# HumanCompatibleAI/overcooked_ai

Measured on NVIDIA H100. Metric: env-steps/sec (joint transitions), higher is better.
Workload: dtype int32

## Files before the change

overcooked_ai_b200/csrc/ovc_rollout.cuh:

```cuda
#pragma once

namespace ovc {

struct Derived {
    uint16_t face[1024];
    uint8_t move[2048];
    int32_t cook5[32];
    int32_t deliver5[32];
    uint8_t potcode5[32][2];
    uint8_t dcode5[32];
    uint8_t pad[32];
};
static_assert(sizeof(Derived) == 4480, "Derived table size");
constexpr int DERIVED_ZERO_CHUNKS = (1024 * 2 + 2048) / 16;
#define OVC_DOFF(field) ((uint32_t)offsetof(Derived, field))
#define OVC_LOFF(field) ((uint32_t)offsetof(ovc_layout_t, field))

constexpr unsigned POT_FROZEN = 1u << 31;
constexpr int ROLLOUT_MAX_STEPS = 1 << 22;

__device__ __forceinline__ unsigned lds_tile(uint32_t a) {
    unsigned v;
    asm volatile("ld.shared.u32 %0, [%1];" : "=r"(v) : "r"(a) : "memory");
    return v;
}
__device__ __forceinline__ void sts_tile(uint32_t a, unsigned v) { asm volatile("st.shared.u32 [%0], %1;" ::"r"(a), "r"(v) : "memory"); }
__device__ __forceinline__ int4 lds_tile4(uint32_t a) {
    int4 v;
    asm volatile("ld.shared.v4.u32 {%0, %1, %2, %3}, [%4];" : "=r"(v.x), "=r"(v.y), "=r"(v.z), "=r"(v.w) : "r"(a) : "memory");
    return v;
}
__device__ __forceinline__ void sts_tile4(uint32_t a, int4 v) {
    asm volatile("st.shared.v4.u32 [%0], {%1, %2, %3, %4};" ::"r"(a), "r"(v.x), "r"(v.y), "r"(v.z), "r"(v.w) : "memory");
}
__device__ __forceinline__ unsigned lds_tbl32(uint32_t a) {
    unsigned v;
    asm volatile("ld.shared.u32 %0, [%1];" : "=r"(v) : "r"(a));
    return v;
}
__device__ __forceinline__ unsigned lds_tbl16(uint32_t a) {
    unsigned short v;
    asm volatile("ld.shared.u16 %0, [%1];" : "=h"(v) : "r"(a));
    return v;
}
__device__ __forceinline__ unsigned lds_tbl8(uint32_t a) {
    unsigned v;
    asm volatile("ld.shared.u8 %0, [%1];" : "=r"(v) : "r"(a));
    return v;
}

__device__ __forceinline__ int recipe_row5(unsigned k5) {
    const int n = k5 & 3;
    const int nt = __popc((k5 >> 2) & ((1u << n) - 1u));
    return ((n - nt) << 2) | nt;
}

__device__ __forceinline__ unsigned code_mask_of(int c) {
    if (c == 0) return 0u;
    if (c <= 6) {
        const int b = (0x0A0005 >> (((c - 1) >> 1) * 8)) & 0xFF;
        return (1u << b) | ((unsigned)((c - 1) & 1) << (b + 1));
    }
    if (c == 7) return 1u << OVC_EV_SOUP_PICKUP;
    if (c <= 13) {
        const int b = (0x0C0207 >> (((c - 8) >> 1) * 8)) & 0xFF;
        return (1u << b) | ((unsigned)((c - 8) & 1) << (b + 1));
    }
    if (c == 14) return 1u << OVC_EV_SOUP_DROP;
    if (c <= 22) {
        const int tom = (c - 15) >> 2, cls = (c - 15) & 3;
        const unsigned base = 1u << (tom ? OVC_EV_POTTING_TOMATO : OVC_EV_POTTING_ONION);
        const unsigned opt = 1u << (OVC_EV_OPTIMAL_ONION_POTTING + tom), via = 1u << (OVC_EV_VIABLE_ONION_POTTING + tom);
        const unsigned cat = 1u << (OVC_EV_CATASTROPHIC_ONION_POTTING + tom), usl = 1u << (OVC_EV_USELESS_ONION_POTTING + tom);
        return base | (cls == 0 ? (opt | via) : cls == 1 ? via : cls == 2 ? cat : (opt | usl));
    }
    const unsigned row = (unsigned)((0xC98654321ull >> ((c - 23) * 4)) & 15u);
    return (1u << OVC_EV_SOUP_DELIVERY) | (row << OVC_EV_RECIPE_SHIFT);
}

template <int S, int SWZ>
struct TileRec {
    uint32_t rec;
    uint32_t xm;
    __device__ __forceinline__ TileRec(uint32_t tile, int tid) {
        rec = tile + (uint32_t)tid * S * 4;
        if (SWZ == 0) xm = 0;
        else if (S <= 32) xm = ((((uint32_t)tid * S * 4) >> 7) & ((1u << SWZ) - 1u)) << 4;
        else xm = (uint32_t)tid * (S / 32);
    }
    __device__ __forceinline__ uint32_t phys(uint32_t off) const {
        if (SWZ == 0) return off;
        if (S <= 32) return off ^ xm;
        return off ^ (((xm + (off >> 7)) & 7u) << 4);
    }
    __device__ __forceinline__ int4 ld4(int c) const { return lds_tile4(rec + phys((uint32_t)c * 16)); }
    __device__ __forceinline__ void st4(int c, int4 v) const { sts_tile4(rec + phys((uint32_t)c * 16), v); }
    __device__ __forceinline__ uint32_t addr(int w) const { return rec + phys((uint32_t)w * 4); }
    __device__ __forceinline__ unsigned ldw(int w) const { return lds_tile(addr(w)); }
    __device__ __forceinline__ void stw(int w, unsigned v) const { sts_tile(addr(w), v); }
};

__device__ __forceinline__ unsigned pot_to_chip(unsigned w, uint32_t D, unsigned clk) {
    const unsigned tp1 = (w >> 8) & 0x3FFFu;
    if ((w & 7u) != OVC_O_SOUP || tp1 == 0) return w & 0x3FFFFFu;
    const unsigned cook = lds_tbl32(D + OVC_DOFF(cook5) + 4u * ((w >> 3) & 31u));
    if (tp1 - 1u > cook) return (w & 0x3FFFFFu) | POT_FROZEN;
    return (w & 0xFFu) | ((clk + (cook - (tp1 - 1u)) + 1u) << 8);
}
__device__ __forceinline__ unsigned pot_to_ext(unsigned w, uint32_t D, unsigned clk) {
    if (w & POT_FROZEN) return w & 0x3FFFFFu;
    const unsigned g = w >> 8;
    if (g == 0) return w;
    const unsigned cook = lds_tbl32(D + OVC_DOFF(cook5) + 4u * ((w >> 3) & 31u));
    const unsigned left = g - 1u > clk ? g - 1u - clk : 0u;
    return (w & 0xFFu) | ((cook - left + 1u) << 8);
}

struct RollOut {
    int sparse, sh0, sh1;
    unsigned c0, c1;
};

constexpr unsigned PS_FULL = 1u, PS_DISH = 1u << 4;
template <class R>
__device__ __forceinline__ unsigned pot_summary(const R &r, int n_pots) {
    unsigned ps = 0;
#pragma unroll 1
    for (int k = 0; k < n_pots; k++) {
        const unsigned w = r.ldw(4 + k);
        const bool soup = (w & 7u) == OVC_O_SOUP;
        const bool idle = (w >> 8) == 0;
        const unsigned n = (w >> 3) & 3u;
        if (soup && (!idle || n == 3u)) ps += PS_FULL;
        if (soup && (!idle || n == 1u || n == 2u)) ps += PS_DISH;
    }
    return ps;
}

template <class R>
__device__ __forceinline__ unsigned interact_v2(const R &r, uint32_t L, uint32_t D, unsigned &me, const unsigned other_t,
                                                unsigned &misc, const unsigned ps, unsigned &psn, const int n_pots,
                                                const bool old_dyn, const unsigned s, int &sparse, int &shaped) {
    const unsigned cell = lds_tbl16(D + OVC_DOFF(face) + 2u * (me & 0x3FFu));
    const unsigned terr = cell & 7u;
    unsigned held = me >> 10;
    const unsigned ht = held & 7u;
    unsigned code = 0;
    if (terr - 1u < 4u) {
        const bool ctr = terr == OVC_T_COUNTER;
        const uint32_t wa = r.addr(4 + (int)(cell >> 8));
        unsigned cw = terr - 1u;
        if (ctr) cw = lds_tile(wa);
        const bool pick = held == 0 && cw != 0;
        const bool drop = ctr && held != 0 && cw == 0;
        if (pick || drop) {
            const unsigned ot = (held | cw) & 7u;
            const unsigned n_full = ps & 15u;
            bool u;
            if (ot == OVC_O_DISH)
                u = pick ? ((misc & 0xFF00u) == 0 && (other_t == OVC_O_DISH ? 1u : 0u) < (ps >> 4)) : (n_full == 0 && other_t != OVC_O_ONION);
            else
                u = ot <= OVC_O_TOMATO && pick != (n_full == (unsigned)n_pots && other_t != OVC_O_DISH);
            code = 2u * ot + (pick ? 0xFFFFFFFFu : 6u) + (unsigned)u;
            if (ctr) {
                sts_tile(wa, held);
                if (ot == OVC_O_DISH) misc += pick ? 0xFFFFFF00u : 0x100u;
            } else {
                if (ot == OVC_O_TOMATO) code = 0;
                if (ot == OVC_O_DISH && u) shaped += (int)lds_tbl32(L + OVC_LOFF(rew_dish_pickup));
            }
            held = pick ? cw : 0u;
        }
    } else if (terr == OVC_T_POT) {
        const uint32_t wa = r.addr(4 + (int)(cell >> 8));
        const unsigned w = lds_tile(wa);
        const unsigned k5 = (w >> 3) & 31u;
        const unsigned n = k5 & 3u;
        if (ht == 0) {
            if (!old_dyn && (w & ~0xF8u) == OVC_O_SOUP && n != 0) {
                sts_tile(wa, w | ((s + lds_tbl32(D + OVC_DOFF(cook5) + 4u * k5) + 1u) << 8));
                psn += n == 3u ? PS_DISH : PS_FULL;
            }
        } else if (ht == OVC_O_DISH) {
            const unsigned g = w >> 8;
            if ((int)w < 0 || g - 1u <= s) {
                code = 7;
                held = pot_to_ext(w, D, s);
                sts_tile(wa, 0u);
                shaped += (int)lds_tbl32(L + OVC_LOFF(rew_soup_pickup));
                psn -= PS_FULL + PS_DISH;
            }
        } else if (ht <= OVC_O_TOMATO) {
            if ((w >> 8) == 0 && n < 3u) {
                const unsigned tom = ht == OVC_O_TOMATO;
                code = lds_tbl8(D + OVC_DOFF(potcode5) + 2u * k5 + tom);
                sts_tile(wa, ((w ? w : (unsigned)OVC_O_SOUP) + 8u) | (tom << (5 + n)));
                shaped += (int)lds_tbl32(L + OVC_LOFF(rew_placement_in_pot));
                held = 0;
                psn += n == 0 ? PS_DISH : n == 2u ? PS_FULL - PS_DISH : 0u;
            }
        }
    } else if (terr == OVC_T_SERVE && ht == OVC_O_SOUP) {
        const unsigned k5 = (held >> 3) & 31u;
        sparse += (int)lds_tbl32(D + OVC_DOFF(deliver5) + 4u * k5);
        code = lds_tbl8(D + OVC_DOFF(dcode5) + k5);
        held = 0;
    }
    me = (me & 0x3FFu) | (held << 10);
    return code;
}

constexpr int FMT_WIDE = 0, FMT_HOST = 1, FMT_STREAM = 2;

template <int FMT>
struct RollIO {
    static constexpr bool WIDE = FMT == FMT_WIDE;
    const StepArgs &a;
    unsigned oi, ai;
    const unsigned n;
    unsigned live_mask, cnt, cap, lane_lt, mi, n_groups;
    unsigned short *vals;
    bool leader;
    __device__ __forceinline__ RollIO(const StepArgs &args, long long env, unsigned live) : a(args), n((unsigned)args.n_envs) {
        oi = ai = (unsigned)env;
        live_mask = live, cnt = 0, cap = 0, lane_lt = 0, mi = 0, n_groups = 0, vals = nullptr, leader = false;
        if (FMT == FMT_STREAM) {
            n_groups = (unsigned)((a.n_envs + 31) >> 5);
            mi = (unsigned)(env >> 5);
            cap = ((unsigned)a.flags >> OVC_F_STREAM_CAP_SHIFT) & 0xFFFFu;
            const unsigned lane = (unsigned)env & 31u;
            lane_lt = (1u << lane) - 1u, leader = lane == 0;
            vals = reinterpret_cast<unsigned short *>(a.sparse) + (size_t)mi * cap;
        }
    }
    __device__ __forceinline__ int2 load_action() const {
        if (!WIDE && (a.flags & OVC_F_ACT_PACKED)) {
            const unsigned u = reinterpret_cast<const unsigned char *>(a.actions)[ai];
            return make_int2((int)(u & 15u), (int)(u >> 4));
        }
        if (!WIDE && (a.flags & OVC_F_ACT_U8)) {
            const uchar2 u = reinterpret_cast<const uchar2 *>(a.actions)[ai];
            return make_int2(u.x, u.y);
        }
        return reinterpret_cast<const int2 *>(a.actions)[ai];
    }
    __device__ __forceinline__ void next_action() { ai += n; }
    __device__ __forceinline__ void write(const RollOut &o, int done_v, bool stepped, uint32_t mask) {
        const unsigned i = oi;
        oi += n;
        if (FMT == FMT_STREAM) {
            const unsigned w = o.c0 | (o.c1 << 5) | ((unsigned)done_v << 10) | (stepped ? 1u << 11 : 0u) |
                               (o.sh0 != 0 ? 1u << 12 : 0u) | (o.sh1 != 0 ? 1u << 13 : 0u);
            const unsigned m = __ballot_sync(live_mask, w != 0);
            if (leader) reinterpret_cast<unsigned *>(a.events)[mi] = m;
            mi += n_groups;
            if (w != 0) {
                const unsigned pos = cnt + __popc(m & lane_lt);
                if (pos < cap) vals[pos] = (unsigned short)w;
            }
            cnt += __popc(m);
            if (a.done) reinterpret_cast<unsigned short *>(a.done)[i] = (unsigned short)w;
            return;
        }
        if (!WIDE && (a.flags & (OVC_F_OUT_CODES | OVC_F_OUT_PACKED))) {
            unsigned w = o.c0 | (o.c1 << 5) | ((unsigned)done_v << 10) | (stepped ? 1u << 11 : 0u);
            if (a.flags & OVC_F_OUT_CODES) {
                w |= (o.sh0 != 0 ? 1u << 12 : 0u) | (o.sh1 != 0 ? 1u << 13 : 0u);
            } else {
                reinterpret_cast<short *>(a.sparse)[i] = (short)o.sparse;
                reinterpret_cast<char2 *>(a.shaped)[i] = make_char2((signed char)o.sh0, (signed char)o.sh1);
            }
            reinterpret_cast<unsigned short *>(a.events)[i] = (unsigned short)w;
            return;
        }
        const unsigned e0 = stepped ? (unsigned)OVC_EVF_STEPPED_DONE : lds_tbl32(mask + 4u * o.c0);
        const unsigned e1 = stepped ? (unsigned)OVC_EVF_STEPPED_DONE : lds_tbl32(mask + 4u * o.c1);
        if (!WIDE && (a.flags & OVC_F_OUT_NARROW)) {
            reinterpret_cast<short *>(a.sparse)[i] = (short)o.sparse;
            reinterpret_cast<unsigned char *>(a.done)[i] = (unsigned char)done_v;
            reinterpret_cast<char2 *>(a.shaped)[i] = make_char2((signed char)o.sh0, (signed char)o.sh1);
        } else {
            a.sparse[i] = o.sparse;
            a.done[i] = done_v;
            reinterpret_cast<int2 *>(a.shaped)[i] = make_int2(o.sh0, o.sh1);
        }
        reinterpret_cast<int2 *>(a.events)[i] = make_int2((int)e0, (int)e1);
    }
};

template <int S, int TILE>
struct RollCfg {
    static constexpr int ROW_WORDS = S == 16 ? 16 : 32;
    static constexpr int ROWS_PER_ENV = S / ROW_WORDS;
    static constexpr int BOX_ROWS = TILE * ROWS_PER_ENV;
    static constexpr int SWZ = S == 16 ? 2 : 3;
    static constexpr int TILE_BYTES = TILE * S * 4;
    static_assert(BOX_ROWS <= 256, "TMA box rows");
    static_assert(TILE_BYTES % 1024 == 0, "tile must keep the swizzle alignment of what follows");
    static size_t smem_bytes(int n_layouts) { return (size_t)TILE_BYTES + (size_t)n_layouts * (sizeof(ovc_layout_t) + sizeof(Derived)) + 128 + 16; }
};

template <int S, int TILE, bool RS, int FMT>
__global__ void __launch_bounds__(TILE)
rollout_kernel(const __grid_constant__ CUtensorMap tmap, const StepArgs a) {
    using C = RollCfg<S, TILE>;
    constexpr bool WIDE = FMT == FMT_WIDE;
    const int tid = threadIdx.x;
    const long long env0 = (long long)blockIdx.x * TILE;
    const long long env = env0 + tid;
    const bool live = env < a.n_envs;
    const int T = a.n_steps;
    const int n_tbl = a.n_layouts;

    extern __shared__ __align__(1024) char smem[];
    char *tile = smem;
    ovc_layout_t *tbl = reinterpret_cast<ovc_layout_t *>(smem + C::TILE_BYTES);
    Derived *der = reinterpret_cast<Derived *>(smem + C::TILE_BYTES + (size_t)n_tbl * sizeof(ovc_layout_t));
    unsigned *mask = reinterpret_cast<unsigned *>(reinterpret_cast<char *>(der) + (size_t)n_tbl * sizeof(Derived));
    uint64_t *bar = reinterpret_cast<uint64_t *>(mask + 32);
    const uint32_t tbl_bytes = (uint32_t)n_tbl * (uint32_t)sizeof(ovc_layout_t);

    if (tid == 0) {
        mbar_init(bar, 1);
        mbar_expect_tx(bar, (uint32_t)C::TILE_BYTES + tbl_bytes);
        prefetch_tmap(&tmap);
        bulk_load_1d(tbl, a.layouts, tbl_bytes, bar);
    }
    for (int l = 0; l < n_tbl; l++)
        for (int i = tid; i < DERIVED_ZERO_CHUNKS; i += TILE) reinterpret_cast<int4 *>(der + l)[i] = make_int4(0, 0, 0, 0);
    if (tid < 32) mask[tid] = code_mask_of(tid);
    asm volatile("griddepcontrol.wait;" ::: "memory");
    if (tid == 0) tma_load_2d(tile, &tmap, 0, (int)(env0 * C::ROWS_PER_ENV), bar);
    int2 act = make_int2(OVC_A_STAY, OVC_A_STAY);
    if (live) act = load_action<WIDE>(a, env);
    __syncthreads();
    mbar_wait(bar, 0);
    asm volatile("griddepcontrol.launch_dependents;" ::: "memory");

    for (int l = 0; l < n_tbl; l++) {
        const ovc_layout_t *L = tbl + l;
        Derived *D = der + l;
        if (tid < 32) {
            const unsigned k5 = tid;
            const int n = k5 & 3, row = recipe_row5(k5);
            D->cook5[k5] = L->cook_time[row];
            D->deliver5[k5] = L->deliver_value[row];
            D->dcode5[k5] = (uint8_t)(23u + (unsigned)((0x0008007605432100ull >> (row * 4)) & 15u));
            const int old_val = L->best_value[n ? row : 0];
#pragma unroll
            for (int tom = 0; tom < 2; tom++) {
                int cls = 0;
                if (n < 3) {
                    const int new_val = L->best_value[recipe_row5((k5 + 1u) | ((unsigned)tom << (2 + n)))];
                    cls = new_val > 0 ? (old_val == new_val ? 0 : 1) : (old_val > 0 ? 2 : 3);
                }
                D->potcode5[k5][tom] = (uint8_t)(15 + 4 * tom + cls);
            }
        }
        const int n_free = L->n_free;
        for (int i = tid; i < n_free * 12; i += TILE) {
            const int f = i / 12, d = i - f * 12;
            const int pos = L->free_pos[f];
            if (d < 4) {
                D->face[(d << 8) | pos] = L->cell[(pos + dir_delta(d)) & 0xFF];
            } else {
                const int act_i = d - 4;
                int np = pos;
                if (act_i < 4) {
                    const int tp = (pos + dir_delta(act_i)) & 0xFF;
                    if ((L->cell[tp] & 7) == OVC_T_FLOOR) np = tp;
                }
                D->move[(act_i << 8) | pos] = (uint8_t)np;
            }
        }
    }
    __syncthreads();

    const unsigned live_mask = __ballot_sync(0xFFFFFFFFu, live);
    if (live) {
        const TileRec<S, C::SWZ> r(smem_u32(tile), tid);
        const uint32_t tbl_s = smem_u32(tbl), der_s = smem_u32(der), mask_s = smem_u32(mask);
        int t;
        unsigned toff;
        unsigned p0, p1, misc, ps, psn;
        uint32_t L, D;
        int n_pots;
        bool old_dyn;
        auto load_regs = [&](unsigned clk) {
            const int4 h = r.ld4(0);
            t = h.x, p0 = (unsigned)h.y, p1 = (unsigned)h.z, misc = (unsigned)h.w;
            toff = clk - (unsigned)t;
            unsigned lid = misc & 0xFFu;
            if (lid >= (unsigned)n_tbl) lid = 0;
            L = tbl_s + lid * (uint32_t)sizeof(ovc_layout_t), D = der_s + lid * (uint32_t)sizeof(Derived);
            n_pots = (int)lds_tbl32(L + OVC_LOFF(n_pots));
            old_dyn = (lds_tbl32(L + OVC_LOFF(flags)) & OVC_LAYOUT_OLD_DYNAMICS) != 0;
#pragma unroll 1
            for (int k = 0; k < n_pots; k++) r.stw(4 + k, pot_to_chip(r.ldw(4 + k), D, clk));
            ps = psn = pot_summary(r, n_pots);
        };
        load_regs(0u);

        RollIO<FMT> io(a, env, live_mask);

        auto interact = [&](bool second, RollOut &o) {
            unsigned pa = second ? p1 : p0;
            const unsigned pb = second ? p0 : p1;
            int sh = 0;
            const unsigned c = interact_v2(r, L, D, pa, (pb >> 10) & 7u, misc, ps, psn, n_pots, old_dyn, (unsigned)t + toff, o.sparse, sh);
            if (second) p1 = pa, o.sh1 = sh, o.c1 = c;
            else p0 = pa, o.sh0 = sh, o.c0 = c;
        };
        auto finish = [&](int a0, int a1, const RollOut &o, bool stepped) {
            int done = 1;
            if (!stepped) {
                const unsigned o0 = p0 & 0xFFu, o1 = p1 & 0xFFu;
                unsigned n0 = lds_tbl8(D + OVC_DOFF(move) + ((((unsigned)a0 & 7u) << 8) | o0));
                unsigned n1 = lds_tbl8(D + OVC_DOFF(move) + ((((unsigned)a1 & 7u) << 8) | o1));
                const bool collide = n0 == n1 || (n0 == o1 && n1 == o0);
                if (collide) n0 = o0, n1 = o1;
                if ((unsigned)a0 < 4u) p0 = (p0 & ~0x3FFu) | ((unsigned)a0 << 8) | n0;
                if ((unsigned)a1 < 4u) p1 = (p1 & ~0x3FFu) | ((unsigned)a1 << 8) | n1;
                if (old_dyn) {
#pragma unroll 1
                    for (int k = 0; k < n_pots; k++) {
                        const unsigned w = r.ldw(4 + k);
                        if ((w & ~0xE0u) == (OVC_O_SOUP | (3u << 3))) {
                            r.stw(4 + k, w | (((unsigned)t + toff + lds_tbl32(D + OVC_DOFF(cook5) + 4u * ((w >> 3) & 31u)) + 1u) << 8));
                            psn += PS_DISH;
                        }
                    }
                }
                ps = psn;
                done = a.horizon > 0 && t + 1 >= a.horizon;
            }
            io.write(o, done, stepped, mask_s);
            if (stepped) return;
            if (done && (a.flags & OVC_F_AUTO_RESET)) {
                const unsigned lid0 = misc & 0xFFu;
                if (RS && a.has_rs) {
                    const unsigned episode = ((misc >> 16) + 1u) & 0xFFFFu;
                    int lid = (int)lid0;
                    if (a.rs.random_layout) lid = random_layout_id(a.rs, (uint64_t)env, episode, a.n_layouts);
                    const ovc_layout_t *Ln = tbl + lid;
                    random_start_record([&](int w, int32_t v) { r.stw(w, (unsigned)v); }, S, a.start_records + (size_t)lid * S,
                                        Ln->cook_time, Ln->free_pos, Ln->n_free, Ln->n_pots, lid, a.rs, (uint64_t)env, episode);
                } else {
                    const int4 *__restrict__ src = reinterpret_cast<const int4 *>(a.start_records + (size_t)lid0 * S);
#pragma unroll 4
                    for (int c = 0; c < S / 4; c++) r.st4(c, __ldg(src + c));
                }
                load_regs((unsigned)t + toff + 1u);
            } else {
                t = t + 1;
            }
        };

        for (int s = 0; s < T; s++) {
            int2 nxt = act;
            io.next_action();
            if (s + 1 < T) nxt = io.load_action();
            const int a0 = act.x, a1 = act.y;
            act = nxt;
            RollOut o{0, 0, 0, 0u, 0u};
            bool stepped = a.horizon > 0 && t >= a.horizon;
            if (FMT != FMT_STREAM) {
                if (stepped) {
                    io.write(o, 1, true, mask_s);
                    continue;
                }
                stepped = false;
            }
            if (!stepped) {
                const bool i0 = a0 == OVC_A_INTERACT, i1 = a1 == OVC_A_INTERACT;
                if (i0 || i1) interact(!i0, o);
                if (i0 && i1) interact(true, o);
            }
            finish(a0, a1, o, FMT == FMT_STREAM && stepped);
        }
#pragma unroll 1
        for (int k = 0; k < n_pots; k++) r.stw(4 + k, pot_to_ext(r.ldw(4 + k), D, (unsigned)t + toff));
        r.st4(0, make_int4(t, (int)p0, (int)p1, (int)misc));
    }
    fence_async_smem();
    __syncthreads();
    if (tid == 0) {
        tma_store_2d(&tmap, 0, (int)(env0 * C::ROWS_PER_ENV), tile);
        bulk_commit();
        bulk_wait_read<0>();
    }
}

}
```

Before: 68.41 billion.

## Table-driven branchless interact with hoisted lookups and deeper action prefetch

Replaces the nested terrain/held-item branching in the interact step with a precomputed per-layout arm table and predicated stores, so warps diverge less. Move, face and arm lookups are hoisted ahead of the interact logic, and the event-mask lookups are skipped when the output format does not need them. Table loads drop asm volatile so the compiler can schedule them, and action loads are prefetched two steps ahead. In exchange the code runs extra speculative shared-memory loads on every step and adds register pressure.

Result: faster. 70.58 billion (median of 6 runs) (+3.2%).

```diff
diff --git a/overcooked_ai_b200/csrc/ovc_rollout.cuh b/overcooked_ai_b200/csrc/ovc_rollout.cuh
--- a/overcooked_ai_b200/csrc/ovc_rollout.cuh
+++ b/overcooked_ai_b200/csrc/ovc_rollout.cuh
@@ -9,9 +9,10 @@
     int32_t deliver5[32];
     uint8_t potcode5[32][2];
     uint8_t dcode5[32];
-    uint8_t pad[32];
+    uint8_t arm[64];
+    int32_t rew[4];
 };
-static_assert(sizeof(Derived) == 4480, "Derived table size");
+static_assert(sizeof(Derived) == 4528, "Derived table size");
 constexpr int DERIVED_ZERO_CHUNKS = (1024 * 2 + 2048) / 16;
 #define OVC_DOFF(field) ((uint32_t)offsetof(Derived, field))
 #define OVC_LOFF(field) ((uint32_t)offsetof(ovc_layout_t, field))
@@ -33,19 +34,22 @@
 __device__ __forceinline__ void sts_tile4(uint32_t a, int4 v) {
     asm volatile("st.shared.v4.u32 [%0], {%1, %2, %3, %4};" ::"r"(a), "r"(v.x), "r"(v.y), "r"(v.z), "r"(v.w) : "memory");
 }
+__device__ __forceinline__ void sts_tile_if(bool p, uint32_t a, unsigned v) {
+    asm volatile("{ .reg .pred p; setp.ne.u32 p, %2, 0; @p st.shared.u32 [%0], %1; }" ::"r"(a), "r"(v), "r"((unsigned)p) : "memory");
+}
 __device__ __forceinline__ unsigned lds_tbl32(uint32_t a) {
     unsigned v;
-    asm volatile("ld.shared.u32 %0, [%1];" : "=r"(v) : "r"(a));
+    asm("ld.shared.u32 %0, [%1];" : "=r"(v) : "r"(a));
     return v;
 }
 __device__ __forceinline__ unsigned lds_tbl16(uint32_t a) {
     unsigned short v;
-    asm volatile("ld.shared.u16 %0, [%1];" : "=h"(v) : "r"(a));
+    asm("ld.shared.u16 %0, [%1];" : "=h"(v) : "r"(a));
     return v;
 }
 __device__ __forceinline__ unsigned lds_tbl8(uint32_t a) {
     unsigned v;
-    asm volatile("ld.shared.u8 %0, [%1];" : "=r"(v) : "r"(a));
+    asm("ld.shared.u8 %0, [%1];" : "=r"(v) : "r"(a));
     return v;
 }
 
@@ -119,6 +123,7 @@
 struct RollOut {
     int sparse, sh0, sh1;
     unsigned c0, c1;
+    unsigned e0, e1;
 };
 
 constexpr unsigned PS_FULL = 1u, PS_DISH = 1u << 4;
@@ -137,76 +142,70 @@
     return ps;
 }
 
+constexpr unsigned ARM_NONE = 0, ARM_CTR = 1,
+    ARM_DISP = 2,
+    ARM_START = 3,
+    ARM_PLATE = 4,
+    ARM_ADD = 5,
+    ARM_SERVE = 6;
+constexpr unsigned ARM_SILENT = 0x80u;
+__device__ __forceinline__ unsigned arm_of(unsigned terr, unsigned ht, bool old_dyn) {
+    if (terr == OVC_T_COUNTER) return ARM_CTR;
+    if (terr - OVC_T_ONION < 3u)
+        return ht ? ARM_NONE : ARM_DISP | (terr - 1u) << 5 | (terr == OVC_T_DISH ? 1u << 3 : 0u) | (terr == OVC_T_TOMATO ? ARM_SILENT : 0u);
+    if (terr == OVC_T_POT) {
+        if (ht == 0) return old_dyn ? ARM_NONE : ARM_START;
+        if (ht == OVC_O_DISH) return ARM_PLATE | 2u << 3;
+        return ht <= OVC_O_TOMATO ? ARM_ADD | 3u << 3 : ARM_NONE;
+    }
+    return terr == OVC_T_SERVE && ht == OVC_O_SOUP ? ARM_SERVE : ARM_NONE;
+}
+
 template <class R>
-__device__ __forceinline__ unsigned interact_v2(const R &r, uint32_t L, uint32_t D, unsigned &me, const unsigned other_t,
-                                                unsigned &misc, const unsigned ps, unsigned &psn, const int n_pots,
-                                                const bool old_dyn, const unsigned s, int &sparse, int &shaped) {
-    const unsigned cell = lds_tbl16(D + OVC_DOFF(face) + 2u * (me & 0x3FFu));
-    const unsigned terr = cell & 7u;
-    unsigned held = me >> 10;
-    const unsigned ht = held & 7u;
+__device__ __forceinline__ unsigned interact_tbl(const R &r, uint32_t D, unsigned &me, const unsigned cell, const unsigned arm,
+                                                 const unsigned other_t, unsigned &misc, const unsigned ps, unsigned &psn,
+                                                 const int n_pots, const unsigned s, int &sparse, int &shaped) {
+    const unsigned cls = arm & 7u;
+    const unsigned held = me >> 10;
+    const uint32_t wa = r.addr(4 + (int)(cell >> 8));
+    const unsigned w = lds_tile(wa);
     unsigned code = 0;
-    if (terr - 1u < 4u) {
-        const bool ctr = terr == OVC_T_COUNTER;
-        const uint32_t wa = r.addr(4 + (int)(cell >> 8));
-        unsigned cw = terr - 1u;
-        if (ctr) cw = lds_tile(wa);
-        const bool pick = held == 0 && cw != 0;
-        const bool drop = ctr && held != 0 && cw == 0;
-        if (pick || drop) {
-            const unsigned ot = (held | cw) & 7u;
-            const unsigned n_full = ps & 15u;
-            bool u;
-            if (ot == OVC_O_DISH)
-                u = pick ? ((misc & 0xFF00u) == 0 && (other_t == OVC_O_DISH ? 1u : 0u) < (ps >> 4)) : (n_full == 0 && other_t != OVC_O_ONION);
-            else
-                u = ot <= OVC_O_TOMATO && pick != (n_full == (unsigned)n_pots && other_t != OVC_O_DISH);
-            code = 2u * ot + (pick ? 0xFFFFFFFFu : 6u) + (unsigned)u;
-            if (ctr) {
-                sts_tile(wa, held);
-                if (ot == OVC_O_DISH) misc += pick ? 0xFFFFFF00u : 0x100u;
-            } else {
-                if (ot == OVC_O_TOMATO) code = 0;
-                if (ot == OVC_O_DISH && u) shaped += (int)lds_tbl32(L + OVC_LOFF(rew_dish_pickup));
-            }
-            held = pick ? cw : 0u;
-        }
-    } else if (terr == OVC_T_POT) {
-        const uint32_t wa = r.addr(4 + (int)(cell >> 8));
-        const unsigned w = lds_tile(wa);
-        const unsigned k5 = (w >> 3) & 31u;
-        const unsigned n = k5 & 3u;
-        if (ht == 0) {
-            if (!old_dyn && (w & ~0xF8u) == OVC_O_SOUP && n != 0) {
-                sts_tile(wa, w | ((s + lds_tbl32(D + OVC_DOFF(cook5) + 4u * k5) + 1u) << 8));
-                psn += n == 3u ? PS_DISH : PS_FULL;
-            }
-        } else if (ht == OVC_O_DISH) {
-            const unsigned g = w >> 8;
-            if ((int)w < 0 || g - 1u <= s) {
-                code = 7;
-                held = pot_to_ext(w, D, s);
-                sts_tile(wa, 0u);
-                shaped += (int)lds_tbl32(L + OVC_LOFF(rew_soup_pickup));
-                psn -= PS_FULL + PS_DISH;
-            }
-        } else if (ht <= OVC_O_TOMATO) {
-            if ((w >> 8) == 0 && n < 3u) {
-                const unsigned tom = ht == OVC_O_TOMATO;
-                code = lds_tbl8(D + OVC_DOFF(potcode5) + 2u * k5 + tom);
-                sts_tile(wa, ((w ? w : (unsigned)OVC_O_SOUP) + 8u) | (tom << (5 + n)));
-                shaped += (int)lds_tbl32(L + OVC_LOFF(rew_placement_in_pot));
-                held = 0;
-                psn += n == 0 ? PS_DISH : n == 2u ? PS_FULL - PS_DISH : 0u;
-            }
-        }
-    } else if (terr == OVC_T_SERVE && ht == OVC_O_SOUP) {
-        const unsigned k5 = (held >> 3) & 31u;
-        sparse += (int)lds_tbl32(D + OVC_DOFF(deliver5) + 4u * k5);
-        code = lds_tbl8(D + OVC_DOFF(dcode5) + k5);
-        held = 0;
-    }
-    me = (me & 0x3FFu) | (held << 10);
+    if (cls - ARM_CTR < 2u) {
+        const bool ctr = cls == ARM_CTR;
+        const unsigned cw = ctr ? w : arm >> 5 & 3u;
+        const bool pick = held == 0;
+        const unsigned ot = (held | cw) & 7u;
+        const unsigned n_full = ps & 15u;
+        const bool u = ot == OVC_O_DISH
+                           ? (pick ? ((misc & 0xFF00u) == 0 && (other_t == OVC_O_DISH ? 1u : 0u) < (ps >> 4)) : (n_full == 0 && other_t != OVC_O_ONION))
+                           : ot <= OVC_O_TOMATO && pick != (n_full == (unsigned)n_pots && other_t != OVC_O_DISH);
+        const bool act = pick != (cw == 0);
+        sts_tile_if(act && ctr, wa, held);
+        if (act && ctr && ot == OVC_O_DISH) misc += pick ? 0xFFFFFF00u : 0x100u;
+        if (act && u && (arm & 0x18u)) shaped += (int)lds_tbl32(D + OVC_DOFF(rew) + 4u * (arm >> 3 & 3u));
+        if (act) code = (arm & ARM_SILENT) ? 0u : 2u * ot + (pick ? 0xFFFFFFFFu : 6u) + (unsigned)u;
+        if (act) me = (me & 0x3FFu) | ((pick ? cw : 0u) << 10);
+    } else if (cls != ARM_NONE) {
+        const bool serve = cls == ARM_SERVE;
+        const unsigned tom = (held & 7u) == OVC_O_TOMATO;
+        const unsigned k5 = ((serve ? held : w) >> 3) & 31u;
+        const unsigned va = lds_tbl32(D + (serve ? OVC_DOFF(deliver5) + 4u * k5 : OVC_DOFF(cook5) + 4u * k5));
+        const unsigned vc = lds_tbl8(D + (serve ? OVC_DOFF(dcode5) + k5 : OVC_DOFF(potcode5) + 2u * k5 + tom));
+        const int rew = (int)lds_tbl32(D + OVC_DOFF(rew) + 4u * (arm >> 3 & 3u));
+        const unsigned n = k5 & 3u, g = w >> 8;
+        const bool start = cls == ARM_START && (w & ~0xF8u) == OVC_O_SOUP && n != 0;
+        const bool plate = cls == ARM_PLATE && ((int)w < 0 || g - 1u <= s);
+        const bool add = cls == ARM_ADD && g == 0 && n < 3u;
+        const unsigned nw = start ? w | ((s + va + 1u) << 8) : add ? ((w ? w : (unsigned)OVC_O_SOUP) + 8u) | (tom << (5 + n)) : 0u;
+        sts_tile_if(start || plate || add, wa, nw);
+        const unsigned soup = (int)w < 0 ? w & 0x3FFFFFu : (w & 0xFFu) | ((va + 1u) << 8);
+        if (plate || add || serve) me = (me & 0x3FFu) | ((plate ? soup : 0u) << 10);
+        if (plate || add || serve) code = plate ? 7u : vc;
+        if (serve) sparse += (int)va;
+        if (plate || add) shaped += rew;
+        const unsigned dps = cls == ARM_START ? 0x10010100u : cls == ARM_PLATE ? 0xEFEFEFEFu : 0x00F10010u;
+        if (start || plate || add) psn += (unsigned)(int)(int8_t)(dps >> (8 * n));
+    }
     return code;
 }
 
@@ -245,7 +244,8 @@
         return reinterpret_cast<const int2 *>(a.actions)[ai];
     }
     __device__ __forceinline__ void next_action() { ai += n; }
-    __device__ __forceinline__ void write(const RollOut &o, int done_v, bool stepped, uint32_t mask) {
+    __device__ __forceinline__ bool wants_masks() const { return WIDE || (FMT == FMT_HOST && !(a.flags & (OVC_F_OUT_CODES | OVC_F_OUT_PACKED))); }
+    __device__ __forceinline__ void write(const RollOut &o, int done_v, bool stepped) {
         const unsigned i = oi;
         oi += n;
         if (FMT == FMT_STREAM) {
@@ -273,8 +273,8 @@
             reinterpret_cast<unsigned short *>(a.events)[i] = (unsigned short)w;
             return;
         }
-        const unsigned e0 = stepped ? (unsigned)OVC_EVF_STEPPED_DONE : lds_tbl32(mask + 4u * o.c0);
-        const unsigned e1 = stepped ? (unsigned)OVC_EVF_STEPPED_DONE : lds_tbl32(mask + 4u * o.c1);
+        const unsigned e0 = stepped ? (unsigned)OVC_EVF_STEPPED_DONE : o.e0;
+        const unsigned e1 = stepped ? (unsigned)OVC_EVF_STEPPED_DONE : o.e1;
         if (!WIDE && (a.flags & OVC_F_OUT_NARROW)) {
             reinterpret_cast<short *>(a.sparse)[i] = (short)o.sparse;
             reinterpret_cast<unsigned char *>(a.done)[i] = (unsigned char)done_v;
@@ -357,12 +357,15 @@
                 D->potcode5[k5][tom] = (uint8_t)(15 + 4 * tom + cls);
             }
         }
+        for (int i = tid; i < 64; i += TILE) D->arm[i] = (uint8_t)arm_of((unsigned)i >> 3, (unsigned)i & 7u, (L->flags & OVC_LAYOUT_OLD_DYNAMICS) != 0);
+        if (tid < 4) D->rew[tid] = tid == 0 ? 0 : tid == 1 ? L->rew_dish_pickup : tid == 2 ? L->rew_soup_pickup : L->rew_placement_in_pot;
         const int n_free = L->n_free;
         for (int i = tid; i < n_free * 12; i += TILE) {
             const int f = i / 12, d = i - f * 12;
             const int pos = L->free_pos[f];
             if (d < 4) {
-                D->face[(d << 8) | pos] = L->cell[(pos + dir_delta(d)) & 0xFF];
+                const unsigned cell = L->cell[(pos + dir_delta(d)) & 0xFF];
+                D->face[(d << 8) | pos] = (uint16_t)((cell >> 8) == OVC_NO_SLOT ? cell & 0xFFu : cell);
             } else {
                 const int act_i = d - 4;
                 int np = pos;
@@ -383,7 +386,7 @@
         int t;
         unsigned toff;
         unsigned p0, p1, misc, ps, psn;
-        uint32_t L, D;
+        uint32_t D;
         int n_pots;
         bool old_dyn;
         auto load_regs = [&](unsigned clk) {
@@ -392,7 +395,8 @@
             toff = clk - (unsigned)t;
             unsigned lid = misc & 0xFFu;
             if (lid >= (unsigned)n_tbl) lid = 0;
-            L = tbl_s + lid * (uint32_t)sizeof(ovc_layout_t), D = der_s + lid * (uint32_t)sizeof(Derived);
+            const uint32_t L = tbl_s + lid * (uint32_t)sizeof(ovc_layout_t);
+            D = der_s + lid * (uint32_t)sizeof(Derived);
             n_pots = (int)lds_tbl32(L + OVC_LOFF(n_pots));
             old_dyn = (lds_tbl32(L + OVC_LOFF(flags)) & OVC_LAYOUT_OLD_DYNAMICS) != 0;
 #pragma unroll 1
@@ -403,20 +407,9 @@
 
         RollIO<FMT> io(a, env, live_mask);
 
-        auto interact = [&](bool second, RollOut &o) {
-            unsigned pa = second ? p1 : p0;
-            const unsigned pb = second ? p0 : p1;
-            int sh = 0;
-            const unsigned c = interact_v2(r, L, D, pa, (pb >> 10) & 7u, misc, ps, psn, n_pots, old_dyn, (unsigned)t + toff, o.sparse, sh);
-            if (second) p1 = pa, o.sh1 = sh, o.c1 = c;
-            else p0 = pa, o.sh0 = sh, o.c0 = c;
-        };
-        auto finish = [&](int a0, int a1, const RollOut &o, bool stepped) {
-            int done = 1;
+        auto finish = [&](int a0, int a1, unsigned n0, unsigned n1, int done, const RollOut &o, bool stepped) {
             if (!stepped) {
                 const unsigned o0 = p0 & 0xFFu, o1 = p1 & 0xFFu;
-                unsigned n0 = lds_tbl8(D + OVC_DOFF(move) + ((((unsigned)a0 & 7u) << 8) | o0));
-                unsigned n1 = lds_tbl8(D + OVC_DOFF(move) + ((((unsigned)a1 & 7u) << 8) | o1));
                 const bool collide = n0 == n1 || (n0 == o1 && n1 == o0);
                 if (collide) n0 = o0, n1 = o1;
                 if ((unsigned)a0 < 4u) p0 = (p0 & ~0x3FFu) | ((unsigned)a0 << 8) | n0;
@@ -432,9 +425,10 @@
                     }
                 }
                 ps = psn;
-                done = a.horizon > 0 && t + 1 >= a.horizon;
-            }
-            io.write(o, done, stepped, mask_s);
+            } else {
+                done = 1;
+            }
+            io.write(o, done, stepped);
             if (stepped) return;
             if (done && (a.flags & OVC_F_AUTO_RESET)) {
                 const unsigned lid0 = misc & 0xFFu;
@@ -456,27 +450,59 @@
             }
         };
 
-        for (int s = 0; s < T; s++) {
-            int2 nxt = act;
-            io.next_action();
-            if (s + 1 < T) nxt = io.load_action();
-            const int a0 = act.x, a1 = act.y;
-            act = nxt;
-            RollOut o{0, 0, 0, 0u, 0u};
+        auto transition = [&](const int a0, const int a1) {
+            RollOut o{0, 0, 0, 0u, 0u, 0u, 0u};
             bool stepped = a.horizon > 0 && t >= a.horizon;
             if (FMT != FMT_STREAM) {
                 if (stepped) {
-                    io.write(o, 1, true, mask_s);
-                    continue;
+                    io.write(o, 1, true);
+                    return;
                 }
                 stepped = false;
             }
-            if (!stepped) {
-                const bool i0 = a0 == OVC_A_INTERACT, i1 = a1 == OVC_A_INTERACT;
-                if (i0 || i1) interact(!i0, o);
-                if (i0 && i1) interact(true, o);
-            }
-            finish(a0, a1, o, FMT == FMT_STREAM && stepped);
+            const unsigned n0 = lds_tbl8(D + OVC_DOFF(move) + ((((unsigned)a0 & 7u) << 8) | (p0 & 0xFFu)));
+            const unsigned n1 = lds_tbl8(D + OVC_DOFF(move) + ((((unsigned)a1 & 7u) << 8) | (p1 & 0xFFu)));
+            const unsigned f0 = lds_tbl16(D + OVC_DOFF(face) + 2u * (p0 & 0x3FFu));
+            const unsigned f1 = lds_tbl16(D + OVC_DOFF(face) + 2u * (p1 & 0x3FFu));
+            const bool i0 = a0 == OVC_A_INTERACT && !stepped, i1 = a1 == OVC_A_INTERACT && !stepped;
+            const unsigned m0 = lds_tbl8(D + OVC_DOFF(arm) + (i0 ? ((f0 & 7u) << 3) | ((p0 >> 10) & 7u) : 0u));
+            const unsigned m1 = lds_tbl8(D + OVC_DOFF(arm) + (i1 ? ((f1 & 7u) << 3) | ((p1 >> 10) & 7u) : 0u));
+            const int done = a.horizon > 0 && t + 1 >= a.horizon;
+            const unsigned clk = (unsigned)t + toff;
+            {
+                unsigned pa = i0 ? p0 : p1;
+                int sh = 0;
+                const unsigned c = interact_tbl(r, D, pa, i0 ? f0 : f1, i0 ? m0 : m1, ((i0 ? p1 : p0) >> 10) & 7u, misc, ps, psn,
+                                                n_pots, clk, o.sparse, sh);
+                if (i0) p0 = pa, o.sh0 = sh, o.c0 = c;
+                else p1 = pa, o.sh1 = sh, o.c1 = c;
+            }
+            if (i0 && i1) {
+                int sh = 0;
+                o.c1 = interact_tbl(r, D, p1, f1, m1, (p0 >> 10) & 7u, misc, ps, psn, n_pots, clk, o.sparse, sh);
+                o.sh1 = sh;
+            }
+            if (io.wants_masks()) o.e0 = lds_tbl32(mask_s + 4u * o.c0), o.e1 = lds_tbl32(mask_s + 4u * o.c1);
+            finish(a0, a1, n0, n1, done, o, FMT == FMT_STREAM && stepped);
+        };
+
+        constexpr int ACT_AHEAD = 2;
+        int2 q[ACT_AHEAD];
+        q[0] = act;
+#pragma unroll
+        for (int k = 1; k < ACT_AHEAD; k++) {
+            io.next_action();
+            q[k] = k < T ? io.load_action() : make_int2(OVC_A_STAY, OVC_A_STAY);
+        }
+        for (int s0 = 0; s0 < T; s0 += ACT_AHEAD) {
+#pragma unroll
+            for (int k = 0; k < ACT_AHEAD; k++) {
+                if (s0 + k >= T) break;
+                const int2 cur = q[k];
+                io.next_action();
+                if (s0 + k + ACT_AHEAD < T) q[k] = io.load_action();
+                transition(cur.x, cur.y);
+            }
         }
 #pragma unroll 1
         for (int k = 0; k < n_pots; k++) r.stw(4 + k, pot_to_ext(r.ldw(4 + k), D, (unsigned)t + toff));
```
